# microsoft/T-MAC

Hardware: AMD Instinct MI355X
Metric: W2A8 GEMV GB/s (llama-2-7B all-layer decode, N=1) (higher is better)
Workload: dtype int8

## Files before the change

include/tmac_hip.h:

```cpp
#ifndef TMAC_HIP_H_
#define TMAC_HIP_H_

#include <stddef.h>
#include <stdint.h>

#ifdef __cplusplus
extern "C" {
#endif
#pragma GCC visibility push(default)

#define TMAC_HIP_OK 0
#define TMAC_HIP_E_NOMATCH (-1)
#define TMAC_HIP_E_NODEVICE (-2)
#define TMAC_HIP_E_RUNTIME (-3)
#define TMAC_HIP_E_ARG (-4)

typedef enum { TMAC_F32 = 0, TMAC_F16 = 1 } tmac_dtype_t;

#define TMAC_HIP_ABI_VERSION 1

typedef struct tmac_kcfg {
    int bm;
    int simd_n_in;
    int simd_n_out;
// ... 102 lines not shown

int32_t tmac_hip_defer(int on);
int32_t tmac_hip_flush(void* stream);
int32_t tmac_hip_defer_stats(uint64_t* flushes, uint64_t* cache_hits, uint64_t* stream_launches, uint64_t* single_calls);

typedef struct tmac_hip_chain tmac_hip_chain;
int32_t tmac_hip_chain_begin(void);
int32_t tmac_hip_chain_begin_independent(void);
int32_t tmac_hip_chain_end(tmac_hip_chain** out);
int32_t tmac_hip_chain_abort(void);
int32_t tmac_hip_chain_launch(tmac_hip_chain* chain, void* stream);
int32_t tmac_hip_chain_status(tmac_hip_chain* chain, uint32_t* error_word);
int32_t tmac_hip_chain_info(const tmac_hip_chain* chain, int op, int32_t* nops, int32_t* wpq, int32_t* grid, size_t* bytes);
int32_t tmac_hip_chain_free(tmac_hip_chain* chain);
#define TMAC_XF_NONE 0
#define TMAC_XF_NORM 1
#define TMAC_XF_GLU 2
#define TMAC_XF_GLU_NORM 4
#define TMAC_XF_GATE_SILU  0x000
#define TMAC_XF_GATE_RELU2 0x100
#define TMAC_XF_GATE_GELU  0x200
#define TMAC_XF_CARRY ((const float*)1)
typedef struct {
    int32_t kind;
    const void* in2;
    const float* residual;
    const float* gamma;
    float eps;
    float* residual_out;
    int32_t keep;
} tmac_hip_xform;
int32_t tmac_hip_chain_xform(const tmac_hip_xform* xf);
int32_t tmac_hip_qgemm_fused_xf_dev(const tmac_hip_weights* const* weights, int nmat, const void* B_dev, tmac_dtype_t act_dtype,
                                    const tmac_hip_xform* xf, void* const* C_dev, tmac_dtype_t out_dtype, void* stream);
int32_t tmac_hip_qgemm_fused_xf_rows_dev(const tmac_hip_weights* const* weights, int nmat, const void* B_dev, tmac_dtype_t act_dtype,
                                         const tmac_hip_xform* xf, void* const* C_dev, tmac_dtype_t out_dtype, int N, void* stream);
int32_t tmac_hip_debug_xf_rows_plan(const tmac_hip_weights* const* weights, int nmat, void* const* C_dev, int N, int32_t* route, int32_t* lut);
int32_t tmac_hip_debug_fused_plan(const tmac_hip_weights* const* weights, int nmat, void* const* C_dev, int N, int32_t* route, int32_t* lut);
int32_t tmac_hip_debug_route_stats(uint64_t counts[8]);
int32_t tmac_hip_debug_xf_rows(const void* B_dev, tmac_dtype_t act_dtype, const tmac_hip_xform* xf, int K, int N, float* x_out_dev,
                               void* stream);
#define TMAC_HIP_CHAIN_BLOB_BYTES 128
int32_t tmac_hip_chain_record_gather(const void* send_dev, void* recv_dev, size_t bytes_per_rank, int rank, int world);
int32_t tmac_hip_chain_export(const tmac_hip_chain* chain, void* blob_out);
int32_t tmac_hip_chain_connect(tmac_hip_chain* chain, const void* blobs_of_all_ranks, int world);
int32_t tmac_hip_chain_threads(void);
int32_t tmac_hip_chain_is_stream(const tmac_hip_chain* chain);
int32_t tmac_hip_chain_set_stamps(tmac_hip_chain* chain, unsigned long long* dev_buffer);
int32_t tmac_hip_chain_set_tap(tmac_hip_chain* chain, int32_t* dev_buffer);
int32_t tmac_hip_chain_tap_layout(const tmac_hip_chain* chain, int op, size_t* offset_ints, size_t* count_ints);
int32_t tmac_hip_debug_chain_config(int force_waves_per_quad, unsigned spin_limit);
int32_t tmac_hip_debug_chain_grid(int workgroups);
int32_t tmac_hip_debug_stream_schedule(const double* items, int n, int grid, int ncls, int target, int lpt, int32_t* out_lo, int32_t* out_w, double* out_load);

#define TMAC_HIP_COMM_ID_BYTES 128
typedef struct tmac_hip_comm tmac_hip_comm;
int32_t tmac_hip_comm_unique_id(void* id_out);
int32_t tmac_hip_comm_init(tmac_hip_comm** out, const void* id, int rank, int world);
int32_t tmac_hip_comm_allgather(tmac_hip_comm* comm, const void* send_dev, void* recv_dev, size_t bytes_per_rank, void* stream);
int32_t tmac_hip_comm_destroy(tmac_hip_comm* comm);
#define TMAC_HIP_COMM_BLOB_BYTES 128
int32_t tmac_hip_comm_init_ipc(tmac_hip_comm** out, size_t max_bytes_per_rank, int rank, int world);
int32_t tmac_hip_comm_export(const tmac_hip_comm* comm, void* blob_out);
int32_t tmac_hip_comm_connect(tmac_hip_comm* comm, const void* blobs_of_all_ranks, int world);
int32_t tmac_hip_comm_status(tmac_hip_comm* comm, uint32_t* error_word);
const char* tmac_hip_comm_last_error(void);

int32_t tmac_hip_workspace_ptrs(tmac_hip_workspace* ws, void** qlut_dev, size_t* nbytes_qlut_per_row,
                                void** lut_scales, void** lut_biases);

int32_t tmac_hip_workspace_read(tmac_hip_workspace* ws, int8_t* qlut_host, float* lut_scales_host,
                                float* lut_biases_host, int K, int N, int act_group_size, void* stream);
int32_t tmac_hip_workspace_write(tmac_hip_workspace* ws, const int8_t* qlut_host, const float* lut_scales_host,
                                 const float* lut_biases_host, int K, int N, int act_group_size, void* stream);
int32_t tmac_hip_qgemm_partial_sums(const tmac_hip_weights* w, const tmac_hip_workspace* ws,
                                    int32_t* PS_host, int N, void* stream);
int32_t tmac_hip_qgemm_fused_partial_sums(const tmac_hip_weights* w, const void* B_dev, tmac_dtype_t act_dtype,
                                          int32_t* PS_host, float* C_host, float* lut_host, int N, void* stream);
int32_t tmac_hip_selftest(const uint32_t* in_host, uint32_t* out_host, int n);
int32_t tmac_hip_selftest_mfma(const uint32_t* in_host, int32_t* out_host);
int32_t tmac_hip_set_variant(int variant);
int32_t tmac_hip_set_gemm_min_n(int n);
int32_t tmac_hip_set_fast_aggregation(int mode);
int32_t tmac_hip_debug_stream_read(const void* dev_src, size_t bytes, void* dev_sink, void* stream);
int32_t tmac_hip_debug_quad_config(int force_threads, int force_waves_per_quad);
int32_t tmac_hip_debug_stamps(unsigned long long* dev_buffer);
int32_t tmac_hip_debug_pairs_min_n(int n);
int32_t tmac_hip_debug_gemm_kernel(int which);
int32_t tmac_hip_debug_gemm_stamps(unsigned long long* dev_buffer);
int32_t tmac_hip_debug_gemm_comb_sums(const tmac_hip_weights* w, const tmac_hip_workspace* ws, int32_t* comb_host, int N, void* stream);
int32_t tmac_hip_debug_gemm_image_read(const tmac_hip_workspace* ws, int8_t* half_tables_host, float* lut_scales_host,
                                       float* lut_biases_host, float* entry_sums_host, int N, void* stream);
int32_t tmac_hip_debug_rows_kernel(int mode);
int32_t tmac_hip_debug_rows_stats(uint64_t* launches);
int32_t tmac_hip_debug_rows_plan(int K, int m_groups, int N, int32_t* r_fit, int32_t* ngroups, int32_t* cap, int32_t* live, size_t* lds_bytes);
int32_t tmac_hip_debug_rows_comb_sums(const tmac_hip_weights* w, const tmac_hip_workspace* ws, int32_t* comb_host, int N, void* stream);
int32_t tmac_hip_debug_host_runs(int on);
int32_t tmac_hip_debug_ws_fill_sync(int on);
int32_t tmac_hip_debug_defer_fail(int nth);
int32_t tmac_hip_autotune_fused(const tmac_hip_weights* const* weights, int nmat, tmac_dtype_t act_dtype,
                                tmac_dtype_t out_dtype, int* best_ft, int* best_wpq, float* best_us, float* heuristic_us);
int32_t tmac_hip_tune_save(const char* path);
int32_t tmac_hip_tune_load(const char* path);
int32_t tmac_hip_tune_clear(void);

int32_t qgemm_lut_int8(int m, int k, int n, int b, void* A, void* LUT, void* Scales, void* LUT_Scales,
// ... 25 lines not shown
```

tmac_amd/binding.py:

```python
from __future__ import annotations

import ctypes as C
import os
import subprocess

HERE = os.path.dirname(os.path.abspath(__file__))
F32, F16 = 0, 1
SRC_F32, SRC_F16, SRC_BF16 = 0, 1, 2
XF_NONE, XF_NORM, XF_GLU, XF_GLU_NORM = 0, 1, 2, 4
XF_GATE_SILU, XF_GATE_RELU2, XF_GATE_GELU = 0x000, 0x100, 0x200


class TMACHipError(RuntimeError):
    def __init__(self, code: int, msg: str):
        super().__init__(f"tmac_hip error {code}: {msg}")
        self.code = code


class XForm(C.Structure):
    _fields_ = [("kind", C.c_int32), ("in2", C.c_void_p), ("residual", C.c_void_p), ("gamma", C.c_void_p), ("eps", C.c_float),
                ("residual_out", C.c_void_p), ("keep", C.c_int32)]


class KCfg(C.Structure):
# ... 89 lines not shown
        "tmac_hip_qgemm_fused_partial_sums": ([vp, vp, C.c_int, vp, vp, vp, C.c_int, vp], i32),
        "tmac_hip_workspace_ptrs": ([vp, C.POINTER(vp), C.POINTER(sz), C.POINTER(vp), C.POINTER(vp)], i32),
        "tmac_hip_workspace_read": ([vp, vp, vp, vp, C.c_int, C.c_int, C.c_int, vp], i32),
        "tmac_hip_workspace_write": ([vp, vp, vp, vp, C.c_int, C.c_int, C.c_int, vp], i32),
        "tmac_hip_qgemm_partial_sums": ([vp, vp, vp, C.c_int, vp], i32),
        "tmac_hip_debug_gemm_kernel": ([C.c_int], i32),
        "tmac_hip_debug_gemm_stamps": ([vp], i32),
        "tmac_hip_debug_gemm_comb_sums": ([vp, vp, vp, C.c_int, vp], i32),
        "tmac_hip_debug_rows_kernel": ([C.c_int], i32),
        "tmac_hip_debug_rows_stats": ([C.POINTER(C.c_uint64)], i32),
        "tmac_hip_debug_rows_plan": ([C.c_int, C.c_int, C.c_int, C.POINTER(C.c_int32), C.POINTER(C.c_int32), C.POINTER(C.c_int32), C.POINTER(C.c_int32), C.POINTER(C.c_size_t)], i32),
        "tmac_hip_debug_rows_comb_sums": ([vp, vp, vp, C.c_int, vp], i32),
        "tmac_hip_debug_gemm_image_read": ([vp, vp, vp, vp, vp, C.c_int, vp], i32),
        "tmac_hip_set_variant": ([C.c_int], i32),
        "tmac_hip_set_gemm_min_n": ([C.c_int], i32),
        "tmac_hip_set_fast_aggregation": ([C.c_int], i32),
        "tmac_hip_debug_stream_read": ([vp, sz, vp, vp], i32),
        "tmac_hip_autotune_fused": ([C.c_void_p, C.c_int, C.c_int, C.c_int, C.POINTER(C.c_int), C.POINTER(C.c_int),
                                     C.POINTER(C.c_float), C.POINTER(C.c_float)], i32),
        "tmac_hip_tune_save": ([C.c_char_p], i32),
        "tmac_hip_tune_load": ([C.c_char_p], i32),
        "tmac_hip_tune_clear": ([], i32),
        "tmac_hip_comm_unique_id": ([vp], i32),
        "tmac_hip_comm_init": ([C.POINTER(vp), vp, C.c_int, C.c_int], i32),
        "tmac_hip_comm_allgather": ([vp, vp, vp, sz, vp], i32),
        "tmac_hip_comm_destroy": ([vp], i32),
        "tmac_hip_comm_init_ipc": ([C.POINTER(vp), sz, C.c_int, C.c_int], i32),
        "tmac_hip_comm_export": ([vp, vp], i32),
        "tmac_hip_comm_connect": ([vp, vp, C.c_int], i32),
        "tmac_hip_comm_status": ([vp, C.POINTER(C.c_uint32)], i32),
        "tmac_hip_comm_last_error": ([], C.c_char_p),
        "tmac_hip_defer": ([C.c_int], i32),
        "tmac_hip_flush": ([vp], i32),
        "tmac_hip_debug_defer_fail": ([C.c_int], i32),
        "tmac_hip_defer_stats": ([C.POINTER(C.c_uint64)] * 4, i32),
        "tmac_hip_chain_begin": ([], i32),
        "tmac_hip_chain_begin_independent": ([], i32),
        "tmac_hip_chain_end": ([C.POINTER(vp)], i32),
        "tmac_hip_chain_launch": ([vp, vp], i32),
        "tmac_hip_chain_status": ([vp, C.POINTER(C.c_uint32)], i32),
        "tmac_hip_chain_info": ([vp, C.c_int, C.POINTER(i32), C.POINTER(i32), C.POINTER(i32), C.POINTER(sz)], i32),
        "tmac_hip_chain_xform": ([C.POINTER(XForm)], i32),
        "tmac_hip_chain_free": ([vp], i32),
        "tmac_hip_chain_set_stamps": ([vp, vp], i32),
        "tmac_hip_chain_set_tap": ([vp, vp], i32),
        "tmac_hip_chain_tap_layout": ([vp, C.c_int, C.POINTER(sz), C.POINTER(sz)], i32),
        "tmac_hip_chain_threads": ([], i32),
        "tmac_hip_chain_is_stream": ([vp], i32),
        "tmac_hip_chain_record_gather": ([vp, vp, sz, C.c_int, C.c_int], i32),
        "tmac_hip_chain_export": ([vp, vp], i32),
        "tmac_hip_chain_connect": ([vp, vp, C.c_int], i32),
        "tmac_hip_debug_chain_grid": ([C.c_int], i32),
        "tmac_hip_debug_stream_schedule": ([C.POINTER(C.c_double), C.c_int, C.c_int, C.c_int, C.c_int, C.c_int, C.POINTER(C.c_int32), C.POINTER(C.c_int32), C.POINTER(C.c_double)], i32),
        "tmac_hip_debug_chain_config": ([C.c_int, C.c_uint], i32),
        "tmac_hip_debug_quad_config": ([C.c_int, C.c_int], i32),
        "tmac_hip_selftest": ([vp, vp, C.c_int], i32),
        "tmac_hip_selftest_mfma": ([vp, vp], i32),
        "tmac_hip_cache_clear": ([], i32),
        "qgemm_lut_int8": ([C.c_int] * 4 + [vp] * 6, i32),
        "preprocessor_int8": ([C.c_int] * 4 + [vp] * 4, i32),
    }
    optional = {"tmac_hip_chain_is_stream", "tmac_hip_chain_begin_independent", "tmac_hip_chain_xform", "tmac_hip_qgemm_fused_xf_dev", "tmac_hip_qgemm_fused_xf_rows_dev", "tmac_hip_debug_xf_rows", "tmac_hip_debug_xf_rows_plan", "tmac_hip_debug_fused_plan", "tmac_hip_debug_route_stats", "tmac_hip_comm_init_ipc", "tmac_hip_comm_export", "tmac_hip_comm_connect", "tmac_hip_comm_status",
                "tmac_hip_ref_blob_bytes", "tmac_hip_pack_gptq_dev", "tmac_hip_pack_codes_dev", "tmac_hip_register_weights_gptq_dev",
                "tmac_hip_register_weights_codes_dev",
                "tmac_hip_absmean_dev", "tmac_hip_pack_absmean_dev", "tmac_hip_register_weights_absmean_dev",
                "tmac_hip_pack_ternary_dev", "tmac_hip_register_weights_ternary_dev", "tmac_hip_debug_pack_ternary_kernel",
                "tmac_hip_kperm_from_gidx_dev", "tmac_hip_kperm_info", "tmac_hip_kperm_read", "tmac_hip_kperm_free", "tmac_hip_weights_kperm_id",
                "tmac_hip_pack_gptq_perm_dev", "tmac_hip_pack_codes_perm_dev", "tmac_hip_register_weights_gptq_perm_dev",
                "tmac_hip_register_weights_codes_perm_dev", "tmac_hip_preprocessor_perm_dev",
                "tmac_hip_debug_rows_kernel", "tmac_hip_debug_rows_stats", "tmac_hip_debug_rows_plan", "tmac_hip_debug_rows_comb_sums"} if os.environ.get("TMAC_HIP_LIB") else set()
    for name, (argt, rest) in sigs.items():
        try:
            fn = getattr(L, name)
        except AttributeError:
            if name in optional:
                continue
            raise
        fn.argtypes, fn.restype = argt, rest
    _lib = L
    return L


def lib() -> C.CDLL:
    return load_library()


def check(rc: int) -> None:
    if rc != 0:
        raise TMACHipError(rc, load_library().tmac_hip_last_error().decode())


def check_count(rc: int) -> int:
    if rc < 0:
        raise TMACHipError(rc, load_library().tmac_hip_last_error().decode())
    return rc
```

tmac_amd/csrc/tmac_chain_host.cpp:

```cpp
#include "tmac_chain_host.h"
#include "tmac_chain_indep.h"
#include <algorithm>
#include <array>
#include <memory>
#include <optional>

using namespace tmac_host;

static thread_local std::vector<ChainRecOp>* g_chain_rec = nullptr;
static thread_local std::vector<ChainRecGather>* g_chain_gat = nullptr;
static thread_local std::optional<XfSpec> g_chain_xf;
static thread_local bool g_chain_declared = false;
bool tmac_host::chain_recording() { return g_chain_rec != nullptr; }
bool tmac_host::chain_recording_independent() { return g_chain_rec != nullptr && g_chain_declared; }
void tmac_host::chain_clear_xform() { g_chain_xf.reset(); }

int32_t tmac_host::chain_record(const FusedCall& c) {
    if (c.N != 1) { chain_clear_xform(); return fail(TMAC_HIP_E_NOMATCH, "a decode chain records N = 1 calls only"); }
    const int32_t nrc = nulls_check(c);
    if (nrc) { chain_clear_xform(); return nrc; }
    ChainRecOp op(c);
    op.perm = c.wl[0]->kperm;
    op.xf = g_chain_xf.value_or(XfSpec{});
    chain_clear_xform();
// ... 112 lines not shown
        for (int cap = ncls; cap >= 1; cap >>= 1) {
            if (pass == 1 && cap != best_cap) continue;
            std::vector<double> load(ncls, 0.0);
            std::vector<std::vector<int>> vis(ncls);
            std::vector<int> order(nop), wof(nop);
            for (int i = 0; i < nop; ++i) {
                int n = 1;
                while (n < cap && items[i] * n / grid < target) n <<= 1;
                order[i] = i; wof[i] = ncls / n;
            }
            if (lpt)
                std::stable_sort(order.begin(), order.end(), [&](int x, int y) {
                    if (wof[x] != wof[y]) return wof[x] > wof[y];
                    return items[x] > items[y];
                });
            for (int oi = 0; oi < nop; ++oi) {
                const int i = order[oi], w = wof[i];
                int bb = 0;
                double bl = 1e300;
                for (int b0 = 0; b0 + w <= ncls; b0 += w) {
                    double m = 0;
                    for (int k = b0; k < b0 + w; ++k) m = load[k] > m ? load[k] : m;
                    if (m < bl) { bl = m; bb = b0; }
                }
                const int wg = cls_lo(bb + w, grid, ncls) - cls_lo(bb, grid, ncls);
                for (int k = bb; k < bb + w; ++k) { load[k] += visit_fixed + items[i] / wg; vis[k].push_back(i); }
                if (pass == 1) { blk_lo[i] = bb; blk_w[i] = w; }
            }
            double span = 0;
            for (int k = 0; k < ncls; ++k) span = load[k] > span ? load[k] : span;
            if (pass == 0 && (best_cap == 0 || span < best_span * 0.999)) { best_span = span; best_cap = cap; }
            if (pass == 1) visits.swap(vis);
        }
    }
}
extern "C" int32_t tmac_hip_debug_stream_schedule(const double* items, int n, int grid, int ncls, int target, int lpt, int32_t* out_lo, int32_t* out_w, double* out_load) {
    if (!items || n < 1 || grid < 1 || ncls < 1 || ncls > 16 || (ncls & (ncls - 1)) || ncls > grid || !out_lo || !out_w) return fail(TMAC_HIP_E_ARG, "bad schedule query");
    std::vector<double> it(items, items + n);
    std::vector<int> lo, w;
    std::vector<std::vector<int>> vis;
    stream_schedule(it, grid, ncls, target, lpt != 0, lo, w, vis);
    for (int i = 0; i < n; ++i) { out_lo[i] = lo[i]; out_w[i] = w[i]; }
    if (out_load)
        for (int k = 0; k < ncls; ++k) {
            out_load[k] = 0;
            for (int i : vis[k]) {
                const int wg = cls_lo(lo[i] + w[i], grid, ncls) - cls_lo(lo[i], grid, ncls);
                out_load[k] += it[i] / wg;
            }
        }
    return TMAC_HIP_OK;
}

static int env_int(const char* name, int dflt) {
    const char* e = getenv(name);
    return e ? atoi(e) : dflt;
}
struct BuildKnobs {
    int wpq = g_knobs.chain_wpq;
    bool glu_epilogue = env_int("TMAC_CHAIN_GLU_EPILOGUE", 1) != 0;
    bool stream = env_int("TMAC_CHAIN_STREAM", 1) != 0;
    int ncls = env_int("TMAC_STREAM_NCLS", 16);
    int visit_items = env_int("TMAC_STREAM_VISIT_ITEMS", 160);
    int qw = env_int("TMAC_STREAM_QW", -1);
    bool lpt = env_int("TMAC_STREAM_LPT", 1) != 0;
    int split = env_int("TMAC_STREAM_SPLIT", 2);
    int split_bits = env_int("TMAC_STREAM_SPLIT_BITS", 3);
    bool split_bits_set = getenv("TMAC_STREAM_SPLIT_BITS") != nullptr;
    int poll_sleep = env_int("TMAC_CHAIN_POLL_SLEEP", 8), poll_delay = env_int("TMAC_CHAIN_POLL_DELAY", 4);
    int issue_first = env_int("TMAC_CHAIN_ISSUE_FIRST", -1), poll_mode = env_int("TMAC_CHAIN_POLL_MODE", 0), poll_grid = env_int("TMAC_CHAIN_POLL_GRID", 0);
    explicit BuildKnobs(int grid) {
        ncls = std::min(std::max(ncls, 1), 16);
        while (ncls > grid || (ncls & (ncls - 1))) --ncls;
    }
};

struct Src { int op, mat; };
struct ChainFlow {
    std::vector<Range> in_r;
    std::vector<std::vector<Range>> out_r;
    std::vector<Src> src, src2;
    std::vector<std::vector<char>> consumed, gathered;
    std::vector<std::vector<char>> dep;
    std::vector<char> epi_of, glu_in_producer;
};
static Src latest_output(const std::vector<ChainRecOp>& rec, const ChainFlow& f, size_t i, const Range& r, const void* p, bool* partial) {
    *partial = false;
    for (size_t j = i; j-- > 0;)
        for (size_t m = 0; m < rec[j].C.size(); ++m)
            if (overlap(r, f.out_r[j][m])) { *partial = rec[j].C[m] != p; return Src{(int)j, (int)m}; }
    return Src{-1, -1};
}
static int32_t analyse_flow(const std::vector<ChainRecOp>& rec, const std::vector<ChainRecGather>& gat, tmac_dtype_t out, ChainFlow& f) {
    const size_t n = rec.size(), out_esz = out == TMAC_F16 ? 2 : 4;
    f.in_r.resize(n); f.out_r.resize(n);
    for (size_t i = 0; i < n; ++i) {
        f.in_r[i] = act_range(rec[i]);
        for (size_t m = 0; m < rec[i].w.size(); ++m) f.out_r[i].push_back(out_range(rec[i], m, out));
        for (size_t m = 0; m < f.out_r[i].size(); ++m)
            for (size_t m2 = 0; m2 < m; ++m2)
                if (overlap(f.out_r[i][m], f.out_r[i][m2])) return fail(TMAC_HIP_E_ARG, "op %zu: outputs %zu and %zu overlap", i, m2, m);
    }
    f.src.assign(n, Src{-1, -1}); f.src2.assign(n, Src{-1, -1});
    f.consumed.resize(n); f.gathered.resize(n);
    for (size_t i = 0; i < n; ++i) { f.consumed[i].assign(rec[i].w.size(), 0); f.gathered[i].assign(rec[i].w.size(), 0); }
    bool partial;
    for (size_t i = 0; i < n; ++i) {
        const ChainRecGather* via = nullptr;
        for (const ChainRecGather& g : gat)
            if (g.pos <= i && g.recv == rec[i].B && (!via || g.pos >= via->pos)) via = &g;
        if (via) {
            for (size_t j = via->pos; j-- > 0 && f.src[i].op < 0;)
                for (size_t m = 0; m < rec[j].C.size(); ++m)
                    if (rec[j].C[m] == via->send) {
                        if (via->bytes != (size_t)rec[j].w[m]->s.Mw * out_esz)
                            return fail(TMAC_HIP_E_ARG, "op %zu: the exchange step gathers %zu bytes per rank, output %zu of op %zu has %zu", i, via->bytes, m, j,
                                        (size_t)rec[j].w[m]->s.Mw * out_esz);
                        if ((size_t)rec[i].w[0]->s.K > (size_t)via->world * rec[j].w[m]->s.Mw)
                            return fail(TMAC_HIP_E_ARG, "op %zu reads %d activations from a gather of %d x %d rows", i, rec[i].w[0]->s.K, via->world, rec[j].w[m]->s.Mw);
                        f.src[i] = Src{(int)j, (int)m};
                        f.consumed[j][m] = 1; f.gathered[j][m] = 1;
                        break;
                    }
            if (f.src[i].op < 0) return fail(TMAC_HIP_E_ARG, "op %zu reads a gathered buffer whose send side no earlier call of the chain writes", i);
            continue;
        }
// ... 209 lines not shown
        const size_t K = (size_t)rec[i].w[0]->s.K;
        if (xf.residual) xf_rd[i].push_back(Range{(const char*)xf.residual, (const char*)xf.residual + K * 4});
        if (xf.in2 && f.src2[i].op < 0) xf_rd[i].push_back(Range{(const char*)xf.in2, (const char*)xf.in2 + K * 2});
        if (xf.gamma) xf_rd[i].push_back(Range{(const char*)xf.gamma, (const char*)xf.gamma + K * 4});
        if (xf.residual_out) xf_wr[i] = Range{(const char*)xf.residual_out, (const char*)xf.residual_out + K * 4};
    }
    for (size_t k = 0; k < n; ++k) {
        for (size_t i = 0; i < n; ++i)
            for (const Range& r : xf_rd[i]) {
                for (size_t m = 0; m < f.out_r[k].size(); ++m)
                    if (overlap(f.out_r[k][m], r) && (i >= k || !all_past(i, k)))
                        return fail(TMAC_HIP_E_NOMATCH, "op %zu writes output %zu over a vector that the transform of op %zu reads from memory and nothing in the "
                                                        "chain orders the writer behind every reader", k, m, i);
                if (xf_wr[k].lo && overlap(xf_wr[k], r) && (i >= k || !all_past(i, k)))
                    return fail(TMAC_HIP_E_NOMATCH, "op %zu: residual_out overlaps a vector that the transform of op %zu reads from memory (a later NORM of the "
                                                    "launch takes the kept vector, TMAC_XF_CARRY)", k, i);
            }
        if (!xf_wr[k].lo) continue;
        for (size_t i = 0; i < n; ++i) {
            if (f.src[i].op < 0 && overlap(xf_wr[k], f.in_r[i]) && (i >= k || !all_past(i, k)))
                return fail(TMAC_HIP_E_NOMATCH, "op %zu: residual_out overlaps activations that op %zu reads from memory", k, i);
            for (size_t m = 0; m < f.out_r[i].size(); ++m)
                if (overlap(xf_wr[k], f.out_r[i][m])) return fail(TMAC_HIP_E_NOMATCH, "op %zu: residual_out overlaps output %zu of op %zu", k, m, i);
            if (i != k && xf_wr[i].lo && overlap(xf_wr[k], xf_wr[i])) return fail(TMAC_HIP_E_NOMATCH, "ops %zu and %zu: overlapping residual_out vectors", i, k);
        }
    }
    return TMAC_HIP_OK;
}

static IndepVerdict independent(const std::vector<ChainRecOp>& rec, const std::vector<ChainRecGather>& gat, const ChainFlow& f) {
    std::vector<IndepOp> io(rec.size());
    for (size_t i = 0; i < rec.size(); ++i) io[i] = IndepOp{f.src[i].op, f.src2[i].op, (int)rec[i].xf.kind, f.epi_of[i]};
    return indep_verdict(io.data(), io.size(), gat.size());
}
static int32_t refuse_declared(const IndepVerdict& v) {
    static const char* const DECL = "the recording was declared independent (tmac_hip_chain_begin_independent)";
    switch (v.why) {
    case INDEP_FLOW: return fail(TMAC_HIP_E_ARG, "op %d reads an output of op %d as its activations: %s", v.op, v.other, DECL);
    case INDEP_FLOW2: return fail(TMAC_HIP_E_ARG, "op %d reads an output of op %d as the second vector of its GLU: %s", v.op, v.other, DECL);
    case INDEP_XFORM: return fail(TMAC_HIP_E_ARG, "op %d carries a vector transform: %s", v.op, DECL);
    case INDEP_EPILOGUE: return fail(TMAC_HIP_E_ARG, "op %d publishes a GLU's product for a later call: %s", v.op, DECL);
    default: return fail(TMAC_HIP_E_ARG, "an exchange step was recorded: %s", DECL);
    }
}
struct StreamPlan {
    std::vector<ChainOp> ops;
    std::vector<size_t> img_off;
    std::vector<int32_t> roles;
    size_t img_bytes = 0, lds_bytes = 0;
    int buf_u4 = 0, max_nst = 0, ncls = 1, vmax = 1, nsplit = 1;
    bool qw = true;
};
static std::optional<StreamPlan> plan_stream(std::vector<ChainOp> ops, int bits, bool g2, int grid, const BuildKnobs& kn) {
    StreamPlan p;
    p.ops = std::move(ops);
    const int nop = (int)p.ops.size(), ncls = p.ncls = kn.ncls;
    p.img_off.resize(nop);
    for (int i = 0; i < nop; ++i) {
        ChainOp& o = p.ops[i];
        o.img_u4 = stream_img_u4(o.K);
        p.img_off[i] = p.img_bytes;
        p.img_bytes += (size_t)o.img_u4 * 16;
        if (o.img_u4 > p.buf_u4) p.buf_u4 = o.img_u4;
        if (o.nst > p.max_nst) p.max_nst = o.nst;
        o.in_gran &= 2;
    }
    const int nwv = STREAM_NLW;
    {
        double it64 = 0, it16 = 0;
        for (const ChainOp& o : p.ops) {
            for (int m = 0; m < o.nmat; ++m) if (((o.m[m].Mw + 3) / 4) % 4) p.qw = false;
            it64 += (double)o.total_q * o.nst; it16 += (double)(o.total_q / 4) * ((o.nu + 15) / 16);
        }
        if (kn.qw == 0 || (kn.qw < 0 && bits >= 3 && it16 > 0.85 * it64)) p.qw = false;
    }
    const bool qw = p.qw;
    auto op_q = [&](const ChainOp& o) { return qw ? o.total_q / 4 : o.total_q; };
    auto op_nst = [&](const ChainOp& o) { return qw ? (o.nu + 15) / 16 : o.nst; };
    std::vector<int> blk_lo, blk_w;
    std::vector<std::vector<int>> visits;
    {
        std::vector<double> items(nop);
        for (int i = 0; i < nop; ++i) items[i] = (double)op_q(p.ops[i]) * op_nst(p.ops[i]);
        stream_schedule(items, grid, ncls, kn.visit_items, kn.lpt, blk_lo, blk_w, visits);
    }
    for (int i = 0; i < nop; ++i) {
        ChainOp& o = p.ops[i];
        const int wlo = cls_lo(blk_lo[i], grid, ncls), wcnt = cls_lo(blk_lo[i] + blk_w[i], grid, ncls) - wlo;
        o.wg_lo = wlo;
        const int tq = op_q(o), nstw = op_nst(o);
        set_wpq(o, (!kn.wpq || nwv % o.wpq || o.wpq > nstw) ? chain_pick_wpq(tq, nstw, wcnt, nwv) : o.wpq, nwv);
        o.q_per = tq / wcnt; o.q_extra = tq % wcnt;
        if (tq / wcnt + 1 + o.ipi >= 4096) return std::nullopt;
        if (qw) for (int m = 0; m < 4; ++m) { if (o.q_end[m] != 0x7fffffff) o.q_end[m] /= 4; o.m[m].q_end /= 4; }
    }
    int vmax = 1;
    for (int k = 0; k < ncls; ++k) if ((int)visits[k].size() > vmax) vmax = (int)visits[k].size();
    p.vmax = vmax;
    const size_t lds2 = stream_lds_bytes(p.buf_u4, (vmax + 1) / 2, qw);
    p.lds_bytes = stream_lds_bytes(p.buf_u4, vmax, qw);
    const int split_bits = (g2 && !kn.split_bits_set && kn.split_bits > 2) ? 2 : kn.split_bits;
    if (kn.split >= 2 && bits <= split_bits && vmax >= 2 && 2 * lds2 + 2048 <= 160 * 1024) { p.nsplit = 2; p.lds_bytes = lds2; }
    for (int ns = 3; ns <= kn.split && ns <= 4; ++ns) {
        const size_t ldsn = stream_lds_bytes(p.buf_u4, (vmax + ns - 1) / ns, qw);
        if (p.nsplit == ns - 1 && vmax >= ns && ns * (ldsn + 1024) <= 160 * 1024) { p.nsplit = ns; p.lds_bytes = ldsn; }
    }
    if (p.lds_bytes > 160 * 1024) return std::nullopt;
    p.roles.assign((size_t)STREAM_ROLE_INTS * ncls * vmax + ncls, 0);
    for (int k = 0; k < ncls; ++k) {
        p.roles[(size_t)STREAM_ROLE_INTS * ncls * vmax + k] = (int32_t)visits[k].size();
        for (size_t v = 0; v < visits[k].size(); ++v) {
            const int i = visits[k][v];
            const ChainOp& o = p.ops[i];
            int32_t* r = p.roles.data() + ((size_t)k * vmax + v) * STREAM_ROLE_INTS;
            const int nstw = op_nst(o);
            r[SR_NST] = nstw; r[SR_IPI] = o.ipi; r[SR_NSG] = o.nsg; r[SR_GSH] = o.gs_shift; r[SR_NU] = o.nu;
            r[SR_QE0] = o.q_end[0]; r[SR_QE1] = o.q_end[1]; r[SR_QE2] = o.q_end[2];
            r[SR_QPER] = o.q_per; r[SR_QEXTRA] = o.q_extra;
            r[SR_IT_LO] = (o.q_per + o.ipi - 1) / o.ipi; r[SR_IT_HI] = (o.q_per + o.ipi) / o.ipi;
            r[SR_TSTRIDE] = o.tstride; r[SR_OP] = i; r[SR_WPQ] = o.wpq; r[SR_WLO] = o.wg_lo;
            for (int wl = 0; wl < STREAM_NLW; ++wl) {
                int32_t* rw = r + SR_COMMON + SRW_INTS * wl;
                const int qs = wl / o.wpq, h = wl - qs * o.wpq;
                auto nq = [&](int cnt) { return qs < cnt ? (cnt - 1 - qs) / o.ipi + 1 : 0; };
                rw[SRW_NQ] = nq(o.q_per) | (nq(o.q_per + 1) << 16);
                rw[SRW_NSTEPS] = h < nstw ? (nstw - h + o.wpq - 1) / o.wpq : 0;
                rw[SRW_H] = h; rw[SRW_QS] = qs;
            }
        }
    }
    return p;
}

static int32_t commit_stream(tmac_hip_chain& c, StreamPlan& p) {
    const size_t role_bytes = p.roles.size() * sizeof(int32_t);
    if (hipMalloc(&c.images, p.img_bytes + role_bytes) != hipSuccess || hipMemset(c.images, 0, p.img_bytes) != hipSuccess ||
        hipMemcpy(static_cast<char*>(c.images) + p.img_bytes, p.roles.data(), role_bytes, hipMemcpyHostToDevice) != hipSuccess)
        return fail(TMAC_HIP_E_RUNTIME, "LUT image allocation failed (%zu bytes)", p.img_bytes + role_bytes);
    c.roles = reinterpret_cast<const int*>(static_cast<char*>(c.images) + p.img_bytes);
    c.nvis = c.roles + (size_t)STREAM_ROLE_INTS * p.ncls * p.vmax;
    c.ncls = p.ncls; c.vmax = p.vmax; c.qw = p.qw; c.nsplit = p.nsplit; c.max_nst = p.max_nst;
    c.ops = std::move(p.ops);
    for (size_t i = 0; i < c.ops.size(); ++i) c.ops[i].img = static_cast<const char*>(c.images) + p.img_off[i];
    c.stream = true; c.buf_u4 = p.buf_u4; c.lds_bytes = p.lds_bytes; c.xforms = 0;
    return TMAC_HIP_OK;
}
static int32_t commit(tmac_hip_chain& c, const ChainLayout& lay) {
    if (!c.stream) {
        c.buf_u4 = chain_buf_u4(lay.maxK);
        c.lds_bytes = chain_lds_bytes(c.buf_u4, (int)c.ops.size(), c.carry_floats + c.tmp_floats + c.gam_floats + c.ext_floats);
        if (c.lds_bytes > 160 * 1024)
            return fail(TMAC_HIP_E_NOMATCH, "%zu calls with K up to %d need %zu bytes of LDS (LUT buffers + call descriptors): record shorter chains",
                        c.ops.size(), lay.maxK, c.lds_bytes);
        ChainArgs probe;
        memset(&probe, 0, sizeof(probe));
        probe.nops = 1;
        int resident = 0;
        hipError_t e = launch_decode_chain(probe, c.bits, c.zp != 0, c.sc_f16 != 0, c.sm, c.g2 != 0, c.grid, c.lds_bytes, nullptr, &resident);
        if (e == hipErrorInvalidValue) return fail(TMAC_HIP_E_NOMATCH, "no decode-chain kernel for this configuration");
        if (e != hipSuccess || resident < 1)
            return fail(TMAC_HIP_E_NOMATCH, "the decode chain's workgroup does not fit a compute unit (%s, %zu bytes of LDS)",
                        e == hipSuccess ? "occupancy 0" : hipGetErrorString(e), c.lds_bytes);
    }
    if (c.arena_bytes) {
        const hipError_t ea = c.world > 1 ? hipExtMallocWithFlags(&c.arena, 2 * c.arena_bytes, hipDeviceMallocFinegrained)
                                          : hipMalloc(&c.arena, 2 * c.arena_bytes);
        if (ea != hipSuccess || hipMemset(c.arena, 0, 2 * c.arena_bytes) != hipSuccess)
            return fail(TMAC_HIP_E_RUNTIME, "hand-off arena allocation failed (%zu bytes)", 2 * c.arena_bytes);
        char* const base = static_cast<char*>(c.arena);
        for (size_t i = 0; i < c.ops.size(); ++i) {
            ChainOp& o = c.ops[i];
            for (int m = 0; m < o.nmat; ++m)
                if (lay.gr[i][m] != NO_IMAGE) o.m[m].GR = reinterpret_cast<uint4*>(base + lay.gr[i][m]);
            if (o.in_gran & 1) o.in = base + lay.in[i];
            if ((o.in_gran & 1) && o.xf_kind == TMAC_XF_GLU) o.in2 = base + lay.in2[i];
        }
    }
    c.connected = c.world == 1;
    if (hipMalloc((void**)&c.d_ops, sizeof(ChainOp) * c.ops.size()) != hipSuccess ||
        hipMemcpy(c.d_ops, c.ops.data(), sizeof(ChainOp) * c.ops.size(), hipMemcpyHostToDevice) != hipSuccess)
        return fail(TMAC_HIP_E_RUNTIME, "descriptor upload failed");
    if (c.has_perm) {
        std::vector<const int32_t*> dp(c.ops.size(), nullptr);
        for (size_t i = 0; i < dp.size(); ++i) if (c.perms[i]) dp[i] = c.perms[i]->dev;
// ... 75 lines not shown
```

Baseline: 6573.

## Add interval-based stream scheduler choosing per-op workgroup ranges by cost model

Adds an alternative host-side scheduler that assigns each op a contiguous workgroup interval of any width, picking count and waves-per-quad from a cost model with a fixed per-visit overhead, instead of power-of-two class blocks. The plan uses intervals only when the modelled span beats the block schedule by a margin, and visits per workgroup are reordered to balance split LDS halves. This aims to reduce load imbalance across workgroups in the persistent stream kernel, at the cost of more planning complexity and a model that may not match the hardware.

Result: no change. 6575, median of 2 (+0.0%).

```diff
diff --git a/include/tmac_hip.h b/include/tmac_hip.h
--- a/include/tmac_hip.h
+++ b/include/tmac_hip.h
@@ -178,6 +178,8 @@
 int32_t tmac_hip_debug_chain_config(int force_waves_per_quad, unsigned spin_limit);
 int32_t tmac_hip_debug_chain_grid(int workgroups);
 int32_t tmac_hip_debug_stream_schedule(const double* items, int n, int grid, int ncls, int target, int lpt, int32_t* out_lo, int32_t* out_w, double* out_load);
+int32_t tmac_hip_debug_stream_intervals(const int32_t* units, const int32_t* steps, int n, int grid, int target, int32_t* out_lo, int32_t* out_cnt,
+                                        int32_t* out_wpq, int64_t* out_load, int64_t* out_model);
 
 #define TMAC_HIP_COMM_ID_BYTES 128
 typedef struct tmac_hip_comm tmac_hip_comm;
diff --git a/tmac_amd/binding.py b/tmac_amd/binding.py
--- a/tmac_amd/binding.py
+++ b/tmac_amd/binding.py
@@ -165,6 +165,7 @@
         "tmac_hip_chain_connect": ([vp, vp, C.c_int], i32),
         "tmac_hip_debug_chain_grid": ([C.c_int], i32),
         "tmac_hip_debug_stream_schedule": ([C.POINTER(C.c_double), C.c_int, C.c_int, C.c_int, C.c_int, C.c_int, C.POINTER(C.c_int32), C.POINTER(C.c_int32), C.POINTER(C.c_double)], i32),
+        "tmac_hip_debug_stream_intervals": ([C.POINTER(C.c_int32), C.POINTER(C.c_int32), C.c_int, C.c_int, C.c_int, C.POINTER(C.c_int32), C.POINTER(C.c_int32), C.POINTER(C.c_int32), C.POINTER(C.c_int64), C.POINTER(C.c_int64)], i32),
         "tmac_hip_debug_chain_config": ([C.c_int, C.c_uint], i32),
         "tmac_hip_debug_quad_config": ([C.c_int, C.c_int], i32),
         "tmac_hip_selftest": ([vp, vp, C.c_int], i32),
@@ -181,7 +182,8 @@
                 "tmac_hip_kperm_from_gidx_dev", "tmac_hip_kperm_info", "tmac_hip_kperm_read", "tmac_hip_kperm_free", "tmac_hip_weights_kperm_id",
                 "tmac_hip_pack_gptq_perm_dev", "tmac_hip_pack_codes_perm_dev", "tmac_hip_register_weights_gptq_perm_dev",
                 "tmac_hip_register_weights_codes_perm_dev", "tmac_hip_preprocessor_perm_dev",
-                "tmac_hip_debug_rows_kernel", "tmac_hip_debug_rows_stats", "tmac_hip_debug_rows_plan", "tmac_hip_debug_rows_comb_sums"} if os.environ.get("TMAC_HIP_LIB") else set()
+                "tmac_hip_debug_rows_kernel", "tmac_hip_debug_rows_stats", "tmac_hip_debug_rows_plan", "tmac_hip_debug_rows_comb_sums",
+                "tmac_hip_debug_stream_intervals"} if os.environ.get("TMAC_HIP_LIB") else set()
     for name, (argt, rest) in sigs.items():
         try:
             fn = getattr(L, name)
diff --git a/tmac_amd/csrc/tmac_chain_host.cpp b/tmac_amd/csrc/tmac_chain_host.cpp
--- a/tmac_amd/csrc/tmac_chain_host.cpp
+++ b/tmac_amd/csrc/tmac_chain_host.cpp
@@ -188,6 +188,195 @@
     return TMAC_HIP_OK;
 }
 
+struct StreamDeal {
+    std::vector<int> lo, cnt, wpq;
+    std::vector<std::vector<int>> visits;
+    int ncls = 1;
+    bool intervals = false;
+};
+constexpr long STREAM_VISIT_FIXED = 10;
+constexpr int STREAM_INTERVAL_GAIN = 10;
+static bool stream_intervals_win(long span_intervals, long span_blocks, int gain_pct) { return span_intervals * 100 <= span_blocks * (100 - gain_pct) && span_intervals < span_blocks; }
+static bool stream_wpq_legal(int wpq, int steps, int nwv) { return wpq >= 1 && wpq <= 4 && nwv % wpq == 0 && (wpq == 1 || wpq <= steps); }
+static long stream_walk_cost(int units, int steps, int cnt, int wpq, int nwv) {
+    const long ipi = nwv / wpq, per = (units + cnt - 1) / cnt;
+    return (long)nwv * ((per + ipi - 1) / ipi) * ((steps + wpq - 1) / wpq);
+}
+static bool stream_wpq_forced(int force, int steps, int nwv) { return force >= 1 && nwv % force == 0 && force <= steps; }
+static int stream_best_wpq(int units, int steps, int cnt, int force, int nwv) {
+    if (stream_wpq_forced(force, steps, nwv)) return force;
+    int best = 1;
+    for (int wpq = 2; wpq <= 4; ++wpq)
+        if (stream_wpq_legal(wpq, steps, nwv) && stream_walk_cost(units, steps, cnt, wpq, nwv) < stream_walk_cost(units, steps, cnt, best, nwv)) best = wpq;
+    return best;
+}
+static long stream_model_span(const std::vector<int>& units, const std::vector<int>& steps, const StreamDeal& d, int grid, int nwv, long fixed, std::vector<long>* load_out = nullptr) {
+    std::vector<long> load(grid, 0);
+    for (size_t i = 0; i < units.size(); ++i) {
+        const long c = stream_walk_cost(units[i], steps[i], d.cnt[i], d.wpq[i], nwv) + fixed;
+        for (int b = d.lo[i]; b < d.lo[i] + d.cnt[i]; ++b) load[b] += c;
+    }
+    long span = 0;
+    for (long l : load) span = std::max(span, l);
+    if (load_out) load_out->swap(load);
+    return span;
+}
+static StreamDeal stream_deal_blocks(const std::vector<int>& units, const std::vector<int>& steps, const std::vector<int>& force, int grid, int ncls, int target, bool lpt, int nwv) {
+    const int nop = (int)units.size();
+    StreamDeal d;
+    d.ncls = ncls; d.lo.resize(nop); d.cnt.resize(nop); d.wpq.resize(nop);
+    std::vector<double> items(nop);
+    for (int i = 0; i < nop; ++i) items[i] = (double)units[i] * steps[i];
+    std::vector<int> blk_lo, blk_w;
+    stream_schedule(items, grid, ncls, target, lpt, blk_lo, blk_w, d.visits);
+    for (int i = 0; i < nop; ++i) {
+        d.lo[i] = cls_lo(blk_lo[i], grid, ncls); d.cnt[i] = cls_lo(blk_lo[i] + blk_w[i], grid, ncls) - d.lo[i];
+        d.wpq[i] = stream_wpq_forced(force[i], steps[i], nwv) ? force[i] : chain_pick_wpq(units[i], steps[i], d.cnt[i], nwv);
+    }
+    return d;
+}
+static bool stream_deal_intervals(const std::vector<int>& units, const std::vector<int>& steps, const std::vector<int>& force, int grid, int target, int nwv, long fixed, StreamDeal& out) {
+    const int nop = (int)units.size();
+    struct Cand { int cnt, wpq; long cost; };
+    std::vector<int> order(nop);
+    for (int i = 0; i < nop; ++i) order[i] = i;
+    std::stable_sort(order.begin(), order.end(), [&](int x, int y) { return (long)units[x] * steps[x] > (long)units[y] * steps[y]; });
+    struct Walk { int units, steps, force; std::vector<Cand> by_cnt; };
+    std::vector<Walk> walks;
+    std::vector<int> walk_of(nop);
+    for (int i = 0; i < nop; ++i) {
+        size_t k = 0;
+        while (k < walks.size() && !(walks[k].units == units[i] && walks[k].steps == steps[i] && walks[k].force == force[i])) ++k;
+        if (k == walks.size()) {
+            Walk wk{units[i], steps[i], force[i], {}};
+            for (int cnt = 1; cnt <= grid && cnt <= units[i]; ++cnt) {
+                const int wpq = stream_best_wpq(units[i], steps[i], cnt, force[i], nwv);
+                if ((units[i] + cnt - 1) / cnt + 1 + nwv / wpq >= 4096) continue;
+                wk.by_cnt.push_back(Cand{cnt, wpq, stream_walk_cost(units[i], steps[i], cnt, wpq, nwv)});
+            }
+            if (wk.by_cnt.empty()) return false;
+            walks.push_back(std::move(wk));
+        }
+        walk_of[i] = (int)k;
+    }
+    long best_span = -1;
+    long all_items = 0;
+    for (int i = 0; i < nop; ++i) all_items += (long)units[i] * steps[i];
+    const long ideal = (all_items + grid - 1) / grid;
+    static const int CAP_DIV[] = {12, 8, 6, 4, 2, 0};
+    constexpr size_t STREAM_MAX_CANDS = 8;
+    std::vector<std::vector<Cand>> prev_cands;
+    for (int div : CAP_DIV) {
+        const long cap = div ? std::max(ideal / div, 1L) : (1L << 60);
+        std::vector<std::vector<Cand>> cands(walks.size());
+        for (size_t k = 0; k < walks.size(); ++k) {
+            const Walk& wk = walks[k];
+            auto area = [&](const Cand& c) { return c.cnt * (c.cost + fixed); };
+            auto fed = [&](const Cand& c) { return (long)((wk.units + c.cnt - 1) / c.cnt) * wk.steps >= target; };
+            int rule = 2;
+            for (const Cand& c : wk.by_cnt) if (c.cost + fixed <= cap) { rule = std::min(rule, fed(c) ? 0 : 1); }
+            const long low = wk.by_cnt.back().cost;
+            auto in_q = [&](const Cand& c) { return rule == 2 ? c.cost == low : (c.cost + fixed <= cap && (rule == 1 || fed(c))); };
+            long best_area = -1;
+            for (const Cand& c : wk.by_cnt) if (in_q(c) && (best_area < 0 || area(c) < best_area)) best_area = area(c);
+            long last_cost = -1;
+            for (const Cand& c : wk.by_cnt) {
+                if (c.cost == last_cost) continue;
+                last_cost = c.cost;
+                if (in_q(c) && area(c) * 97 <= best_area * 100) cands[k].push_back(c);
+            }
+            if (cands[k].size() > STREAM_MAX_CANDS) {
+                std::vector<Cand> by_area = cands[k];
+                std::stable_sort(by_area.begin(), by_area.end(), [&](const Cand& x, const Cand& y) { return area(x) < area(y); });
+                const long worst = area(by_area[STREAM_MAX_CANDS - 1]);
+                std::vector<Cand> kept;
+                for (const Cand& c : cands[k]) if (area(c) <= worst && kept.size() < STREAM_MAX_CANDS) kept.push_back(c);
+                cands[k].swap(kept);
+            }
+        }
+        auto same = [](const std::vector<Cand>& x, const std::vector<Cand>& y) {
+            if (x.size() != y.size()) return false;
+            for (size_t j = 0; j < x.size(); ++j) if (x[j].cnt != y[j].cnt || x[j].wpq != y[j].wpq) return false;
+            return true;
+        };
+        bool repeat = !prev_cands.empty();
+        for (size_t k = 0; repeat && k < walks.size(); ++k) repeat = same(cands[k], prev_cands[k]);
+        if (repeat) continue;
+        prev_cands = cands;
+        StreamDeal d;
+        d.ncls = grid; d.intervals = true; d.lo.assign(nop, 0); d.cnt.assign(nop, 1); d.wpq.assign(nop, 1);
+        d.visits.assign(grid, std::vector<int>());
+        std::vector<long> load(grid, 0), pre(grid + 1, 0);
+        std::vector<int> dq(grid);
+        for (int oi = 0; oi < nop; ++oi) {
+            const int i = order[oi];
+            for (int b = 0; b < grid; ++b) pre[b + 1] = pre[b] + load[b];
+            long b_top = -1, b_idle = 0, b_area = 0;
+            int b_lo = 0;
+            const Cand* b_c = nullptr;
+            for (const Cand& c : cands[walk_of[i]]) {
+                const long h = c.cost + fixed, area = c.cnt * h;
+                int qh = 0, qt = 0;
+                for (int b = 0; b < grid; ++b) {
+                    while (qt > qh && load[dq[qt - 1]] <= load[b]) --qt;
+                    dq[qt++] = b;
+                    const int lo = b - c.cnt + 1;
+                    if (lo < 0) continue;
+                    if (dq[qh] < lo) ++qh;
+                    const long mx = load[dq[qh]], top = mx + h, idle = mx * c.cnt - (pre[b + 1] - pre[lo]);
+                    if (b_top < 0 || top < b_top || (top == b_top && (idle < b_idle || (idle == b_idle && area < b_area)))) {
+                        b_top = top; b_idle = idle; b_area = area; b_lo = lo; b_c = &c;
+                    }
+                }
+            }
+            d.lo[i] = b_lo; d.cnt[i] = b_c->cnt; d.wpq[i] = b_c->wpq;
+            for (int b = b_lo; b < b_lo + b_c->cnt; ++b) { load[b] += b_c->cost + fixed; d.visits[b].push_back(i); }
+        }
+        const long span = stream_model_span(units, steps, d, grid, nwv, fixed);
+        if (best_span < 0 || span < best_span) { best_span = span; out = std::move(d); }
+    }
+    return true;
+}
+static void stream_order_visits(const std::vector<int>& units, const std::vector<int>& steps, StreamDeal& d, int nsplit, int nwv, long fixed) {
+    if (nsplit < 2) return;
+    for (std::vector<int>& vis : d.visits) {
+        auto cost = [&](int i) { return stream_walk_cost(units[i], steps[i], d.cnt[i], d.wpq[i], nwv) + fixed; };
+        std::stable_sort(vis.begin(), vis.end(), [&](int x, int y) { return cost(x) > cost(y); });
+        std::vector<long> part_load(nsplit, 0);
+        std::vector<int> parts(nsplit), slot(vis.size());
+        for (size_t v0 = 0; v0 < vis.size(); v0 += nsplit) {
+            for (int p = 0; p < nsplit; ++p) parts[p] = p;
+            std::stable_sort(parts.begin(), parts.end(), [&](int x, int y) { return part_load[x] < part_load[y]; });
+            const size_t n = std::min(vis.size() - v0, (size_t)nsplit);
+            if (n < (size_t)nsplit) { std::vector<int> low(parts.begin(), parts.end()); parts.clear(); for (int p : low) if ((size_t)p < n) parts.push_back(p); }
+            for (size_t k = 0; k < n; ++k) { slot[v0 + parts[k]] = vis[v0 + k]; part_load[parts[k]] += cost(vis[v0 + k]); }
+        }
+        vis.swap(slot);
+    }
+}
+extern "C" int32_t tmac_hip_debug_stream_intervals(const int32_t* units, const int32_t* steps, int n, int grid, int target, int32_t* out_lo, int32_t* out_cnt,
+                                                   int32_t* out_wpq, int64_t* out_load, int64_t* out_model) {
+    if (!units || !steps || n < 1 || grid < 1 || !out_lo || !out_cnt || !out_wpq) return fail(TMAC_HIP_E_ARG, "bad schedule query");
+    for (int i = 0; i < n; ++i) if (units[i] < 1 || steps[i] < 1) return fail(TMAC_HIP_E_ARG, "bad schedule query");
+    const std::vector<int> u(units, units + n), s(steps, steps + n), force(n, 0);
+    StreamDeal d;
+    if (!stream_deal_intervals(u, s, force, grid, target, STREAM_NLW, STREAM_VISIT_FIXED, d)) return fail(TMAC_HIP_E_NOMATCH, "a call has too many row units for any number of ranges");
+    std::vector<long> load;
+    const long span = stream_model_span(u, s, d, grid, STREAM_NLW, STREAM_VISIT_FIXED, &load);
+    for (int i = 0; i < n; ++i) { out_lo[i] = d.lo[i]; out_cnt[i] = d.cnt[i]; out_wpq[i] = d.wpq[i]; }
+    if (out_load) for (int b = 0; b < grid; ++b) out_load[b] = load[b];
+    if (out_model) {
+        int ncls = 16;
+        while (ncls > grid) ncls >>= 1;
+        const StreamDeal blk = stream_deal_blocks(u, s, force, grid, ncls, target, true, STREAM_NLW);
+        long items = 0;
+        for (int i = 0; i < n; ++i) items += (long)u[i] * s[i];
+        out_model[0] = span; out_model[1] = stream_model_span(u, s, blk, grid, STREAM_NLW, STREAM_VISIT_FIXED); out_model[2] = (items + grid - 1) / grid;
+        out_model[3] = STREAM_VISIT_FIXED; out_model[4] = STREAM_NLW; out_model[5] = stream_intervals_win(out_model[0], out_model[1], STREAM_INTERVAL_GAIN);
+    }
+    return TMAC_HIP_OK;
+}
+
 static int env_int(const char* name, int dflt) {
     const char* e = getenv(name);
     return e ? atoi(e) : dflt;
@@ -197,6 +386,10 @@
     bool glu_epilogue = env_int("TMAC_CHAIN_GLU_EPILOGUE", 1) != 0;
     bool stream = env_int("TMAC_CHAIN_STREAM", 1) != 0;
     int ncls = env_int("TMAC_STREAM_NCLS", 16);
+    bool ncls_set = getenv("TMAC_STREAM_NCLS") != nullptr;
+    int sched = 0;
+    long visit_fixed = env_int("TMAC_STREAM_VISIT_FIXED", (int)STREAM_VISIT_FIXED);
+    int iv_gain = env_int("TMAC_STREAM_IV_GAIN", STREAM_INTERVAL_GAIN);
     int visit_items = env_int("TMAC_STREAM_VISIT_ITEMS", 160);
     int qw = env_int("TMAC_STREAM_QW", -1);
     bool lpt = env_int("TMAC_STREAM_LPT", 1) != 0;
@@ -208,6 +401,7 @@
     explicit BuildKnobs(int grid) {
         ncls = std::min(std::max(ncls, 1), 16);
         while (ncls > grid || (ncls & (ncls - 1))) --ncls;
+        if (const char* e = getenv("TMAC_STREAM_SCHED")) sched = !strcmp(e, "blocks") ? 1 : !strcmp(e, "intervals") ? 2 : 0;
     }
 };
 
@@ -523,50 +717,48 @@
     bool qw = true;
 };
 static std::optional<StreamPlan> plan_stream(std::vector<ChainOp> ops, int bits, bool g2, int grid, const BuildKnobs& kn) {
-    StreamPlan p;
-    p.ops = std::move(ops);
-    const int nop = (int)p.ops.size(), ncls = p.ncls = kn.ncls;
-    p.img_off.resize(nop);
+    StreamPlan base;
+    base.ops = std::move(ops);
+    const int nop = (int)base.ops.size();
+    base.img_off.resize(nop);
     for (int i = 0; i < nop; ++i) {
-        ChainOp& o = p.ops[i];
+        ChainOp& o = base.ops[i];
         o.img_u4 = stream_img_u4(o.K);
-        p.img_off[i] = p.img_bytes;
-        p.img_bytes += (size_t)o.img_u4 * 16;
-        if (o.img_u4 > p.buf_u4) p.buf_u4 = o.img_u4;
-        if (o.nst > p.max_nst) p.max_nst = o.nst;
+        base.img_off[i] = base.img_bytes;
+        base.img_bytes += (size_t)o.img_u4 * 16;
+        if (o.img_u4 > base.buf_u4) base.buf_u4 = o.img_u4;
+        if (o.nst > base.max_nst) base.max_nst = o.nst;
         o.in_gran &= 2;
     }
     const int nwv = STREAM_NLW;
     {
         double it64 = 0, it16 = 0;
-        for (const ChainOp& o : p.ops) {
-            for (int m = 0; m < o.nmat; ++m) if (((o.m[m].Mw + 3) / 4) % 4) p.qw = false;
+        for (const ChainOp& o : base.ops) {
+            for (int m = 0; m < o.nmat; ++m) if (((o.m[m].Mw + 3) / 4) % 4) base.qw = false;
             it64 += (double)o.total_q * o.nst; it16 += (double)(o.total_q / 4) * ((o.nu + 15) / 16);
         }
-        if (kn.qw == 0 || (kn.qw < 0 && bits >= 3 && it16 > 0.85 * it64)) p.qw = false;
-    }
-    const bool qw = p.qw;
+        if (kn.qw == 0 || (kn.qw < 0 && bits >= 3 && it16 > 0.85 * it64)) base.qw = false;
+    }
+    const bool qw = base.qw;
     auto op_q = [&](const ChainOp& o) { return qw ? o.total_q / 4 : o.total_q; };
     auto op_nst = [&](const ChainOp& o) { return qw ? (o.nu + 15) / 16 : o.nst; };
-    std::vector<int> blk_lo, blk_w;
-    std::vector<std::vector<int>> visits;
-    {
-        std::vector<double> items(nop);
-        for (int i = 0; i < nop; ++i) items[i] = (double)op_q(p.ops[i]) * op_nst(p.ops[i]);
-        stream_schedule(items, grid, ncls, kn.visit_items, kn.lpt, blk_lo, blk_w, visits);
-    }
+    std::vector<int> units(nop), steps(nop), force(nop);
+    for (int i = 0; i < nop; ++i) { units[i] = op_q(base.ops[i]); steps[i] = op_nst(base.ops[i]); force[i] = kn.wpq ? base.ops[i].wpq : 0; }
+    auto build = [&](StreamDeal d) -> std::optional<StreamPlan> {
+    StreamPlan p = base;
+    const int ncls = p.ncls = d.ncls;
     for (int i = 0; i < nop; ++i) {
         ChainOp& o = p.ops[i];
-        const int wlo = cls_lo(blk_lo[i], grid, ncls), wcnt = cls_lo(blk_lo[i] + blk_w[i], grid, ncls) - wlo;
+        const int wlo = d.lo[i], wcnt = d.cnt[i];
         o.wg_lo = wlo;
-        const int tq = op_q(o), nstw = op_nst(o);
-        set_wpq(o, (!kn.wpq || nwv % o.wpq || o.wpq > nstw) ? chain_pick_wpq(tq, nstw, wcnt, nwv) : o.wpq, nwv);
+        const int tq = units[i];
+        set_wpq(o, d.wpq[i], nwv);
         o.q_per = tq / wcnt; o.q_extra = tq % wcnt;
         if (tq / wcnt + 1 + o.ipi >= 4096) return std::nullopt;
         if (qw) for (int m = 0; m < 4; ++m) { if (o.q_end[m] != 0x7fffffff) o.q_end[m] /= 4; o.m[m].q_end /= 4; }
     }
     int vmax = 1;
-    for (int k = 0; k < ncls; ++k) if ((int)visits[k].size() > vmax) vmax = (int)visits[k].size();
+    for (int k = 0; k < ncls; ++k) if ((int)d.visits[k].size() > vmax) vmax = (int)d.visits[k].size();
     p.vmax = vmax;
     const size_t lds2 = stream_lds_bytes(p.buf_u4, (vmax + 1) / 2, qw);
     p.lds_bytes = stream_lds_bytes(p.buf_u4, vmax, qw);
@@ -577,6 +769,8 @@
         if (p.nsplit == ns - 1 && vmax >= ns && ns * (ldsn + 1024) <= 160 * 1024) { p.nsplit = ns; p.lds_bytes = ldsn; }
     }
     if (p.lds_bytes > 160 * 1024) return std::nullopt;
+    if (d.intervals) stream_order_visits(units, steps, d, p.nsplit, nwv, kn.visit_fixed);
+    const std::vector<std::vector<int>>& visits = d.visits;
     p.roles.assign((size_t)STREAM_ROLE_INTS * ncls * vmax + ncls, 0);
     for (int k = 0; k < ncls; ++k) {
         p.roles[(size_t)STREAM_ROLE_INTS * ncls * vmax + k] = (int32_t)visits[k].size();
@@ -601,6 +795,16 @@
         }
     }
     return p;
+    };
+    StreamDeal blocks = stream_deal_blocks(units, steps, force, grid, kn.ncls, kn.visit_items, kn.lpt, nwv), intervals;
+    const bool blocks_forced = kn.sched == 1 || (kn.sched == 0 && kn.ncls_set);
+    const bool have_iv = !blocks_forced && stream_deal_intervals(units, steps, force, grid, kn.visit_items, nwv, kn.visit_fixed, intervals);
+    const bool iv_first = have_iv && (kn.sched == 2 || stream_intervals_win(stream_model_span(units, steps, intervals, grid, nwv, kn.visit_fixed),
+                                                                          stream_model_span(units, steps, blocks, grid, nwv, kn.visit_fixed), kn.iv_gain));
+    std::optional<StreamPlan> plan;
+    if (iv_first) plan = build(std::move(intervals));
+    if (!plan) plan = build(std::move(blocks));
+    return plan;
 }
 
 static int32_t commit_stream(tmac_hip_chain& c, StreamPlan& p) {
```
